# mbrzus/Cross-Modality-Minipig-Gan

Measured on AMD Instinct MI355X. Metric: T1->T2 256x256 slices/sec (G+D step), higher is better.
Workload: dtype f32

## Files before the change

### cross-modality-minipig-gan_amd/csrc/loss_ops.hip

```cpp
#include "mpgan_common.h"

namespace mpgan {

constexpr int LIN_CHUNKS = 64;
constexpr int L1_PARTIALS = 1024;

static inline int ew_blocks2(long total) {
  long b = (total + 255) / 256;
  if (b > 4096) b = 4096;
  if (b < 1) b = 1;
  return (int)b;
}

__device__ __forceinline__ float block_sum_256(float v, float* sh) {
  v = wave_sum(v);
  const int lane = threadIdx.x & 63, w = threadIdx.x >> 6;
  if (lane == 0) sh[w] = v;
  __syncthreads();
  float r = sh[0] + sh[1] + sh[2] + sh[3];
  __syncthreads();
  return r;
}

__global__ __launch_bounds__(256) void linear1_partial_kernel(const float* __restrict__ z, Pro p, long P, int C,
// ... 174 lines not shown
  sh[threadIdx.x] = s;
  __syncthreads();
  if (threadIdx.x == 0) {
    double t = 0.0;
    for (int i = 0; i < 256; ++i) t += sh[i];
    *loss = (float)(t * inv_numel);
  }
}

__global__ __launch_bounds__(256) void adam_kernel(float* __restrict__ p, const float* __restrict__ g,
                                                   float* __restrict__ m, float* __restrict__ v, long numel,
                                                   float w1, float b2, float one_minus_b2, float step_size,
                                                   float bc2_sqrt, float eps, float gscale) {
  const long stride = (long)gridDim.x * blockDim.x;
  for (long i = (long)blockIdx.x * blockDim.x + threadIdx.x; i < numel; i += stride) {
    const float gi = g[i] * gscale;
    float mi = m[i], vi = v[i];
    const float diff = gi - mi;
    mi = w1 < 0.5f ? mi + w1 * diff : gi - diff * (1.f - w1);
    vi = vi * b2 + one_minus_b2 * gi * gi;
    const float denom = sqrtf(vi) / bc2_sqrt + eps;
    p[i] = p[i] - step_size * (mi / denom);
    m[i] = mi;
    v[i] = vi;
  }
}

__global__ __launch_bounds__(256) void pack_weights_kernel(const float* __restrict__ src, float* __restrict__ dst,
                                                           const int64_t* __restrict__ table) {
  const int64_t* e = table + (long)blockIdx.y * 8;
  const long so = e[0], dof = e[1];
  const int Cout = (int)e[2], Cin = (int)e[3], T = (int)e[4];
  const int transposed = (int)e[5], dgrad = (int)e[6];
  const long total = (long)Cout * Cin * T;
  const long stride = (long)gridDim.x * blockDim.x;
  for (long i = (long)blockIdx.x * blockDim.x + threadIdx.x; i < total; i += stride) {
    int co, ci, t;
    if (dgrad == 0) {
      ci = (int)(i % Cin);
      long q = i / Cin;
      t = (int)(q % T);
      co = (int)(q / T);
    } else if (dgrad == 1) {
      co = (int)(i % Cout);
      long q = i / Cout;
      t = (int)(q % T);
      ci = (int)(q / T);
    } else {
      co = (int)(i % Cout);
      long q = i / Cout;
      ci = (int)(q % Cin);
      t = (int)(q / Cin);
    }
    const long s = transposed ? ((long)ci * Cout + co) * T + t : ((long)co * Cin + ci) * T + t;
    dst[dof + i] = src[so + s];
  }
}

__global__ __launch_bounds__(256) void add_tanh_kernel(const float* __restrict__ a, const float* __restrict__ b,
                                                       long numel, int apply_tanh, float* __restrict__ y) {
  const long stride = (long)gridDim.x * blockDim.x;
  for (long i = (long)blockIdx.x * blockDim.x + threadIdx.x; i < numel; i += stride) {
    float v = a[i] + (b ? b[i] : 0.f);
    y[i] = apply_tanh ? tanhf(v) : v;
  }
}

__global__ __launch_bounds__(256) void tanh_backward_kernel(const float* __restrict__ g, const float* __restrict__ y,
                                                            long numel, float* __restrict__ dx) {
  const long stride = (long)gridDim.x * blockDim.x;
  for (long i = (long)blockIdx.x * blockDim.x + threadIdx.x; i < numel; i += stride) {
    const float t = y[i];
    dx[i] = g[i] * (1.f - t * t);
  }
}

__global__ __launch_bounds__(256) void axpby_kernel(const float* __restrict__ a, float alpha,
                                                    const float* __restrict__ b, float beta, long numel,
                                                    float* __restrict__ y) {
  const long stride = (long)gridDim.x * blockDim.x;
  for (long i = (long)blockIdx.x * blockDim.x + threadIdx.x; i < numel; i += stride)
    y[i] = alpha * a[i] + (b ? beta * b[i] : 0.f);
}

struct PatchGeom {
  int B, D, H, W, S, rz, ry, rx;
};

// ... 217 lines not shown
```

### cross-modality-minipig-gan_amd/engine.py

```python
from __future__ import annotations

import ctypes as C
import dataclasses
import math
import os
import struct
from typing import List, Optional, Sequence, Tuple

import torch
import torch.nn as nn

from . import ops
from ._lib import lib
from .ops import ACT_LEAKY, ACT_NONE, ConvGeom, Prologue


class KernelProbe:

    def __init__(self, want=None, detail=False, min_flops=0.0):
        self.want = want
        self.detail = detail
        self.min_flops = min_flops
        self.samples = []

# ... 184 lines not shown
def gather_kernel_name(g: ConvGeom, backward_data: bool, has_pro: bool, per_sample_norm: bool = False,
                       fast_leaky: bool = False) -> str:
    gc = g.c()
    pro = (2 if per_sample_norm else (3 if fast_leaky else 1)) if has_pro else 0
    return kernel_label(lib().mpgan_conv_kernel_name, C.byref(gc), int(backward_data), pro)


def wgrad_kernel_name(g: ConvGeom, pro=None, bf16_dy: bool = False) -> str:
    gc = g.c()
    code = (2 if pro.n_stride else (3 if _fast_leaky(pro) else 1)) if pro is not None else 0
    return kernel_label(lib().mpgan_conv_wgrad_kernel_name, C.byref(gc), code, int(bf16_dy))


def kernel_label(entry, *args) -> str:
    buf = C.create_string_buffer(160)
    if entry(*args, buf, len(buf)):
        raise RuntimeError(lib().mpgan_last_error().decode())
    return buf.value.decode()


def _ld(t):
    return 0 if t is None else ops._cl(t, "plan tensor")[2]


def _p(t):
    return None if t is None else t.data_ptr()


class ConvRec:
    __slots__ = ("mod", "transposed", "cout", "cin", "taps", "w_off", "fwd_off", "bwd_off", "tco", "tco_off")


class FusedRec:
    __slots__ = ("a", "b", "w_off", "b_off", "cout", "cin", "taps")


class ParamStore:

    def __init__(self, module: nn.Module):
        self.module = module
        self.convs: List[ConvRec] = []
        self.fused: List[FusedRec] = []
        self._by_mod = {}
        self.flat = None
        self.flat_grad = None
        self.packed = None
        self.table = None
        self.version = 0
        self.frozen = False
        self._touched = 0
        self._pack_state = {}
        self.flatten()
        for m in module.modules():
            if isinstance(m, (nn.Conv2d, nn.Conv3d, nn.ConvTranspose2d, nn.ConvTranspose3d)):
                tr = isinstance(m, (nn.ConvTranspose2d, nn.ConvTranspose3d))
                self.register_conv(m, cout=m.out_channels, cin=m.in_channels, taps=math.prod(m.kernel_size), transposed=tr)

    def flatten(self):
        params = list(self.module.parameters())
        dev = params[0].device
        offs, total = [], 0
        for p in params:
            total = (total + 3) // 4 * 4
            offs.append(total)
            total += p.numel()
        total = (total + 3) // 4 * 4
        flat = torch.zeros(total, dtype=torch.float32, device=dev)
# ... 43 lines not shown
            assert (r.cout, r.cin, r.taps, r.transposed) == (cout, cin, taps, transposed)
            return r
        if self.frozen:
            raise RuntimeError("ParamStore: conv registered after plans were built")
        r = ConvRec()
        r.mod, r.transposed, r.cout, r.cin, r.taps = mod, transposed, cout, cin, taps
        r.tco, r.tco_off = tco, -1
        self.convs.append(r)
        self._by_mod[id(mod)] = r
        if self.flat is not None:
            self._build_pack_table()
        return r

    def register_fused(self, conv_a, conv_b) -> FusedRec:
        for f in self.fused:
            if f.a.mod is conv_a and f.b.mod is conv_b:
                return f
        if self.frozen:
            raise RuntimeError("ParamStore: fused pair registered after plans were built")
        ra, rb = self._by_mod[id(conv_a)], self._by_mod[id(conv_b)]
        assert (ra.cin, ra.taps, ra.transposed, rb.transposed) == (rb.cin, rb.taps, False, False)
        assert conv_a.bias is not None and conv_b.bias is not None
        f = FusedRec()
        f.a, f.b, f.cout, f.cin, f.taps = ra, rb, ra.cout + rb.cout, ra.cin, ra.taps
        self.fused.append(f)
        self._build_pack_table()
        return f

    def wp_fused(self, f: FusedRec) -> torch.Tensor:
        return self.packed[f.w_off:f.w_off + f.cout * f.cin * f.taps]

    def bias_fused(self, f: FusedRec) -> torch.Tensor:
        return self.packed[f.b_off:f.b_off + f.cout]

    def _build_pack_table(self):
        if not self.convs:
            return
        rows, off = [], 0
        for r in self.convs:
            n = r.cout * r.cin * r.taps
            assert r.mod.weight.numel() == n, (r.mod, n)
            r.w_off = self.offset(r.mod.weight)
            r.fwd_off = off
            off += (n + 3) // 4 * 4
            r.bwd_off = off
            off += (n + 3) // 4 * 4
            rows.append([r.w_off, r.fwd_off, r.cout, r.cin, r.taps, int(r.transposed), 0, 0])
            rows.append([r.w_off, r.bwd_off, r.cout, r.cin, r.taps, int(r.transposed), 1, 0])
            if r.tco:
                r.tco_off = off
                off += (n + 3) // 4 * 4
                rows.append([r.w_off, r.tco_off, r.cout, r.cin, r.taps, int(r.transposed), 2, 0])
        for f in self.fused:
            na, nb_ = f.a.cout * f.cin * f.taps, f.b.cout * f.cin * f.taps
            f.w_off = off
            rows.append([f.a.w_off, off, f.a.cout, f.cin, f.taps, 0, 0, 0])
            rows.append([f.b.w_off, off + na, f.b.cout, f.cin, f.taps, 0, 0, 0])
            off += (na + nb_ + 3) // 4 * 4
            f.b_off = off
            rows.append([self.offset(f.a.mod.bias), off, f.a.cout, 1, 1, 0, 0, 0])
            rows.append([self.offset(f.b.mod.bias), off + f.a.cout, f.b.cout, 1, 1, 0, 0, 0])
            off += (f.cout + 3) // 4 * 4
        dev = self.flat.device
        self.packed = torch.empty(off, dtype=torch.float32, device=dev)
        self.table = torch.tensor(rows, dtype=torch.int64, device=dev)
        self._max_elems = max(r.cout * r.cin * r.taps for r in self.convs)
        self._pack_state.clear()

    def emit_pack(self, prog: Program):
        self.frozen = True
        fn = lib().mpgan_pack_weights
        args = (self.flat.data_ptr(), self.packed.data_ptr(), self.table.data_ptr(), self.table.shape[0], self._max_elems)
        state = self._pack_state
        packed_params = [r.mod.weight for r in self.convs]
        for f in self.fused:
            packed_params += [f.a.mod.bias, f.b.mod.bias]

        def pack_if_stale(stream):
            key = (self.flat._version, self.version, self._touched, sum(p._version for p in packed_params))
            if state.get("key") == key and not _ALWAYS_PACK:
                return 0
            rc = fn(*args, stream)
            if rc == 0:
                state["key"] = key
            return rc

        prog.add("pack_weights", pack_if_stale, keep=(self.flat, self.packed, self.table))

    def touch(self):
        self._touched += 1

    def wp(self, rec: ConvRec) -> torch.Tensor:
        return self.packed[rec.fwd_off:rec.fwd_off + rec.cout * rec.cin * rec.taps]

    def wp_bwd(self, rec: ConvRec) -> torch.Tensor:
# ... 784 lines not shown
        gcat_last = G["gcat"][L - 2]
        g_b = gcat_last[..., bt["cb_in"]:]
        gd_last = gcat_last[..., :bt["cb_in"]]
        d_last = cats[L - 2][..., :bt["cb_in"]]
        dzb1, gab0 = G["dzb1"], G["gab0"]
        emit_norm_bwd(b, g_b, bt["zb1"], bt["nbb1"], prelu_pro(bt["nbb1"], bt["BA1"]), dzb1, part,
                      gv(bt["BN1"].weight), gv(bt["BN1"].bias), gv(bt["BA1"].weight))
        emit_conv_wgrad(bw, bt["gb1"], bt["zb0"], dzb1, gv(bt["bc1"].weight), ws, pro=prelu_pro(bt["nbb0"], bt["BA0"]),
                        dbias=gv(bt["bc1"].bias), lane=1)
        emit_conv_dgrad(b, bt["gb1"], dzb1, wpb(R(bt["bc1"])), gab0)
        emit_norm_bwd(b, gab0, bt["zb0"], bt["nbb0"], prelu_pro(bt["nbb0"], bt["BA0"]), gab0, part,
                      gv(bt["BN0"].weight), gv(bt["BN0"].bias), gv(bt["BA0"].weight))
        emit_conv_wgrad(bw, bt["gb0"], d_last, gab0, gv(bt["bc0"].weight), ws, dbias=gv(bt["bc0"].bias), lane=1)
        emit_conv_dgrad(b, bt["gb0"], gab0, wpb(R(bt["bc0"])), gd_last, resid=gd_last)
        if bt["res"] is not None:
            emit_conv_wgrad(bw, bt["gbr"], d_last, g_b, gv(bt["res"].weight), ws, dbias=gv(bt["res"].bias), lane=1)
            emit_conv_dgrad(b, bt["gbr"], g_b, wpb(R(bt["res"])), gd_last, resid=gd_last)
        else:
            emit_norm_act_add(b, g_b, None, gd_last, None, gd_last)
        for l in range(L - 2, -1, -1):
            s = down_state[l]
            (cv0, N0, A0), (cv1, N1, A1) = s["ru"].units
            g_d = G["gcat"][l][..., :s["c"]]
            dz1, ga0 = G["dz1"][l], G["ga0"][l]
            emit_norm_bwd(b, g_d, s["z1"], s["nb1"], prelu_pro(s["nb1"], A1), dz1, part, gv(N1.weight), gv(N1.bias),
                          gv(A1.weight))
            emit_conv_wgrad(bw, s["g1"], s["z0"], dz1, gv(cv1.weight), ws, pro=prelu_pro(s["nb0"], A0),
                            dbias=gv(cv1.bias), lane=1)
            emit_conv_dgrad(b, s["g1"], dz1, wpb(R(cv1)), ga0)
            emit_norm_bwd(b, ga0, s["z0"], s["nb0"], prelu_pro(s["nb0"], A0), ga0, part, gv(N0.weight), gv(N0.bias),
                          gv(A0.weight))
            emit_conv_wgrad(bw, s["g0"], s["xin"], ga0, gv(cv0.weight), ws, dbias=gv(cv0.bias), lane=1)
            emit_conv_wgrad(bw, s["gr"], s["xin"], g_d, gv(s["ru"].res.weight), ws, dbias=gv(s["ru"].res.bias), lane=1)
            if l > 0:
                tgt = G["gcat"][l - 1][..., :chans[l - 1]]
                emit_conv_dgrad(b, s["g0"], ga0, wpb(R(cv0)), tgt, resid=tgt)
                emit_conv_dgrad(b, s["gr"], g_d, wpb(R(s["ru"].res)), tgt, resid=tgt)
            elif g_x is not None:
                emit_conv_dgrad(b, s["g0"], ga0, wpb(R(cv0)), g_x)
                emit_conv_dgrad(b, s["gr"], g_d, wpb(R(s["ru"].res)), g_x, resid=g_x)
        b.extend(bw)
        if own_mark is not None:
            b.mark(own_mark)
        else:
            b.join()


class GeneratorPlan:

    def __init__(self, gen, store: ParamStore, n: int, spatial: Sequence[int], *, want_backward: bool,
                 want_input_grad: bool, instance: bool, training: bool = True, mm_bf16: bool = False):
        self.mm_bf16 = mm_bf16
        unets = [m for m in gen.model if not isinstance(m, nn.Tanh)]
        dims = unets[0].dimensions
        dev = store.flat.device
        dhw = _t3(spatial, dims, 1)
        self.n, self.dhw, self.dims = n, dhw, dims
        self.store = store
        E = lambda *shape: torch.empty(*shape, device=dev)
        self.acts = [E(n, *dhw, 1) for _ in range(len(unets) + 1)]
        self.x_in, self.y = self.acts[0], self.acts[-1]
        self.scratch = Scratch(dev)
        self.want_backward = want_backward
        chans = list(unets[0].channels)
        L = len(chans)
        gb = None
        if want_backward:
            sizes = [dhw]
            for l in range(L - 1):
                sizes.append(tuple((s + 1) // 2 if i >= 3 - dims else s for i, s in enumerate(sizes[-1])))
            in_ch = [1] + chans[:L - 2]
            sub_out = [chans[l] for l in range(L - 2)] + [chans[L - 1]]
            def grad_scratch():
                return dict(
                    gcat=[E(n, *sizes[l + 1], chans[l] + sub_out[l]) for l in range(L - 1)],
                    dzu=[E(n, *sizes[l], in_ch[l]) for l in range(L - 1)],
                    gta=[E(n, *sizes[l], in_ch[l]) for l in range(L - 1)],
                    dz1=[E(n, *sizes[l + 1], chans[l]) for l in range(L - 1)],
                    ga0=[E(n, *sizes[l + 1], chans[l]) for l in range(L - 1)],
                    dzb1=E(n, *sizes[L - 1], chans[L - 1]), gab0=E(n, *sizes[L - 1], chans[L - 1]))
            gb = [grad_scratch(), grad_scratch()]
            self.g_acts = [E(n, *dhw, 1) for _ in range(len(unets) + 1)]
            self.g_y = E(n, *dhw, 1)
        self.unet_plans: List[UNetPlan] = []
        nU = len(unets)
        marks = [Mark() for _ in range(nU)]
        for u, unet in enumerate(unets):
            g = None
            if want_backward:
                g = dict(gb[u % 2])
                g["g_out"] = self.g_acts[u + 1]
                g["g_x"] = self.g_acts[u] if (u > 0 or want_input_grad) else None
            with geom_defaults(mm_bf16=mm_bf16):
                self.unet_plans.append(UNetPlan(unet, store, n, spatial, self.acts[u], self.acts[u + 1],
                                                tanh_out=(u == nU - 1), instance=instance, want_backward=want_backward,
                                                gbufs=g, scratch=self.scratch, training=training,
                                                own_mark=marks[u], wait_mark=marks[u + 2] if u + 2 < nU else None))
        self.scratch.alloc()
        wants = [w for p in self.unet_plans for w in p.acc_wants]
        self.acc_all = None
        if wants:
            total = sum(ops.ACC_REPLICAS * ops.ACC_WORDS * cw for _, cw in wants)
            self.acc_all = torch.zeros(total, dtype=torch.int64, device=dev)
            off = 0
            for nb, cw in wants:
                sz = ops.ACC_REPLICAS * ops.ACC_WORDS * cw
                nb.acc = self.acc_all[off:off + sz]
                off += sz
        for p in self.unet_plans:
            p.emit()
        self.fwd = Program()
        store.emit_pack(self.fwd)
# ... 481 lines not shown
```

### cross-modality-minipig-gan_amd/csrc/conv_igemm.hip

```cpp
#include "mpgan_common.h"
#include "conv_geom.h"
#include "lds_dma.h"
#include "conv_pipe.h"
#include <stdlib.h>
#include <algorithm>
#include <type_traits>

namespace mpgan {


struct KCursor {
  int ci, jz, jy, jx;
  int delta;
  int dz, dy, dx;
  int woff;
  bool valid;
};

template <int BN, int TM, int TN, int WN, bool SCALAR>
__global__ __launch_bounds__(256) void gather_conv_kernel(const GatherConv p) {
  extern __shared__ __attribute__((aligned(16))) float lds[];
  constexpr int STAGE = (BM + BN) * PITCH;
  constexpr int BROWS = BN / 32;

// ... 673 lines not shown
        if ((unsigned)iy >= (unsigned)p.Hi) continue;
        const long rowbase = (((long)d.n * p.Di + iz) * p.Hi + iy) * p.Wi;
        for (int jx = 0; jx < ph.nx; ++jx) {
          const int ix = d.bx + ph.dx0 + p.dstep[2] * jx, kx = ph.kx0 + p.kstep[2] * jx;
          if ((unsigned)ix >= (unsigned)p.Wi) continue;
          float4 v;
          if constexpr (IN_BF16) {
            typedef __bf16 bf16x4 __attribute__((ext_vector_type(4)));
            const bf16x4 t = *reinterpret_cast<const bf16x4*>(reinterpret_cast<const __bf16*>(p.in) + (rowbase + ix) * p.ldi + 4 * l);
            v = make_float4((float)t[0], (float)t[1], (float)t[2], (float)t[3]);
          } else {
            v = *reinterpret_cast<const float4*>(p.in + (rowbase + ix) * p.ldi + 4 * l);
          }
          const float4 w = *reinterpret_cast<const float4*>(wl + ((kz * p.Ky + ky) * p.Kx + kx) * p.Cin + 4 * l);
          acc = fmaf(v.x, w.x, acc);
          acc = fmaf(v.y, w.y, acc);
          acc = fmaf(v.z, w.z, acc);
          acc = fmaf(v.w, w.w, acc);
        }
      }
    }
  }
#pragma unroll
  for (int off = LANES / 2; off > 0; off >>= 1) acc += __shfl_xor(acc, off, 64);
  if (live && d.opix >= 0 && l == 0) {
    float v = acc + (p.bias ? p.bias[0] : 0.f);
    if (p.epi.scale) v = epi_act1(v, p.epi.scale[0], p.epi.shift[0], p.epi.slope[0]);
    if (p.resid) v += p.resid[(long)d.opix * p.ldr];
    if (p.tanh_out) v = tanhf(v);
    p.out[(long)d.opix * p.ldo] = v;
  }
}

template <int LANES>
__global__ __launch_bounds__(256) void convt_quad_cout1_kernel(const GatherConv p) {
  extern __shared__ __attribute__((aligned(16))) float wl[];
  const int Cin = p.Cin;
  for (int i = threadIdx.x; i < 9 * Cin; i += 256) wl[i] = p.wp[i];
  __syncthreads();
  const Phase& ph = p.ph[0];
  const unsigned Mtot = (unsigned)p.N * p.Hi * p.Wi;
  const unsigned gi = blockIdx.x * 256u + threadIdx.x;
  const unsigned m = gi / LANES;
  const int l = (int)(gi % LANES);
  const bool live = m < Mtot;
  unsigned q, ux, uy;
  fdivmod(live ? m : 0u, ph.fMx, q, ux);
  fdivmod(q, ph.fMy, q, uy);
  const int n = (int)q, y = (int)uy, x = (int)ux;
  const float* base = p.in + ((long)(n * p.Hi + y) * p.Wi + x) * p.ldi + 4 * l;
  const bool y1 = y + 1 < p.Hi, x1 = x + 1 < p.Wi;
  const float4 z4 = make_float4(0.f, 0.f, 0.f, 0.f);
  const float4 v00 = live ? *reinterpret_cast<const float4*>(base) : z4;
  const float4 v01 = live && x1 ? *reinterpret_cast<const float4*>(base + p.ldi) : z4;
  const float4 v10 = live && y1 ? *reinterpret_cast<const float4*>(base + (long)p.Wi * p.ldi) : z4;
  const float4 v11 = live && y1 && x1 ? *reinterpret_cast<const float4*>(base + (long)(p.Wi + 1) * p.ldi) : z4;
  auto W = [&](int ky, int kx) { return *reinterpret_cast<const float4*>(wl + (ky * 3 + kx) * Cin + 4 * l); };
  auto dot = [](const float4& a, const float4& b, float acc) {
    acc = fmaf(a.x, b.x, acc); acc = fmaf(a.y, b.y, acc); acc = fmaf(a.z, b.z, acc); return fmaf(a.w, b.w, acc);
  };
  float o00 = dot(v00, W(1, 1), 0.f);
  float o01 = dot(v01, W(1, 0), dot(v00, W(1, 2), 0.f));
  float o10 = dot(v10, W(0, 1), dot(v00, W(2, 1), 0.f));
  float o11 = dot(v11, W(0, 0), dot(v10, W(0, 2), dot(v01, W(2, 0), dot(v00, W(2, 2), 0.f))));
  const bool b0 = l & 1, b1 = l & 2;
  const float r0 = (b0 ? o10 : o00) + __shfl_xor(b0 ? o00 : o10, 1, 64);
// ... 232 lines not shown

static bool thin_c1c1_ok(const GatherConv& p) {
  static const bool off = dev_env("MPGAN_DBG_NO_THIN_ROWS") != nullptr;
  if (off || !(p.Cin == 1 && p.Cout == 1 && p.ldi == 1 && p.ldo == 1 && (!p.resid || p.ldr == 1) && p.nphase == 1 &&
               !p.pro.scale && !p.stats && !p.stats_acc && !p.in_bf16 && !p.out_bf16 && !p.epi.scale && p.Ky == 3 && p.Kx == 3 &&
               (p.Kz == 3 || p.Kz == 1)))
    return false;
  const Phase& ph = p.ph[0];
  if (!(ph.ny == 3 && ph.nx == 3 && ph.nz == p.Kz && ph.oz == 0 && ph.oy == 0 && ph.ox == 0 && p.Do == ph.Mz &&
        p.Ho == ph.My && p.Wo == ph.Mx && p.Wi == ph.Mx && p.Hi == ph.My && p.Di == ph.Mz))
    return false;
  for (int d = 0; d < 3; ++d) {
    if (p.istride[d] != 1 || p.ostride[d] != 1) return false;
    if (d == 0 && p.Kz == 1) continue;
    const int d0 = d == 0 ? ph.dz0 : (d == 1 ? ph.dy0 : ph.dx0);
    if (!((p.dstep[d] == 1 && d0 == -1) || (p.dstep[d] == -1 && d0 == 1))) return false;
  }
  return true;
}

static bool thin_cin1_ok(const GatherConv& p) {
  const int T = p.Kz * p.Ky * p.Kx;
  return p.Cin == 1 && !p.pro.scale && (long)T * ((p.Cout + 3) / 4 * 4) * 4 <= 48 * 1024;
}

static bool thin_cout1_ok(const GatherConv& p) {
  const int T = p.Kz * p.Ky * p.Kx;
  const int lanes = p.Cin / 4;
  return p.Cout == 1 && !p.pro.scale && p.Cin % 4 == 0 && p.ldi % 4 == 0 && lanes >= 1 && lanes <= 64 &&
         (lanes & (lanes - 1)) == 0 && ((reinterpret_cast<uintptr_t>(p.in) & 15) == 0) &&
         (long)T * p.Cin * 4 <= 48 * 1024;
}

template <int T, bool OUT_BF16>
__global__ __launch_bounds__(256) void thin_cin1_rows_kernel(const GatherConv p) {
  __shared__ float red[4][128];
  constexpr int KZ = T == 27 ? 3 : 1;
  const Phase& ph = p.ph[0];
  const int lane = threadIdx.x & 63;
  const int wave = __builtin_amdgcn_readfirstlane((int)threadIdx.x >> 6);
  const int rows = p.N * ph.Mz * ph.My, Mx = ph.Mx;
  const int nwaves = (int)gridDim.x * 4, ngroups = (Mx + 3) >> 2;
  float w[T];
#pragma unroll
  for (int t = 0; t < T; ++t) w[t] = p.wp[(long)lane * T + t];
  const float bv = p.bias ? p.bias[lane] : 0.f;
  const bool act = OUT_BF16 && p.epi.scale != nullptr;
  const float esc = act ? p.epi.scale[lane] : 1.f, esh = act ? p.epi.shift[lane] : 0.f, esl = act ? p.epi.slope[lane] : 1.f;
  float s1 = 0.f, s2 = 0.f;
  for (int r = (int)blockIdx.x * 4 + wave; r < rows; r += nwaves) {
    const int my = r % ph.My, q = r / ph.My;
    const int mz = q % ph.Mz, n = q / ph.Mz;
    const float* __restrict__ g0 = p.in + (((long)n * p.Di + mz) * p.Hi + my) * p.Wi;
    const long orow = (long)r * Mx;
    for (int gi = 0; gi < ngroups; ++gi) {
      const int x0 = gi + 1 < ngroups ? 4 * gi : Mx - 4;
      const int first = 4 * gi - x0;
      float o[4] = {bv, bv, bv, bv};
#pragma unroll
      for (int kz = 0; kz < KZ; ++kz)
#pragma unroll
        for (int ky = 0; ky < 3; ++ky) {
          const float* __restrict__ src = g0 + ((long)kz * p.Hi + ky) * p.Wi + x0;
          float win[6];
#pragma unroll
          for (int i = 0; i < 6; ++i) win[i] = src[i];
#pragma unroll
          for (int kx = 0; kx < 3; ++kx)
#pragma unroll
            for (int j = 0; j < 4; ++j) o[j] = fmaf(w[(kz * 3 + ky) * 3 + kx], win[j + kx], o[j]);
        }
#pragma unroll
      for (int j = 0; j < 4; ++j) {
        const long e = (orow + x0 + j) * p.ldo + lane;
        if constexpr (OUT_BF16) reinterpret_cast<__bf16*>(p.out)[e] = (__bf16)(act ? epi_act1(o[j], esc, esh, esl) : o[j]);
        else p.out[e] = o[j];
        const float v = j >= first ? o[j] : 0.f;
        s1 += v;
        s2 = fmaf(v, v, s2);
      }
    }
  }
  if (p.stats) {
    red[wave][lane] = s1;
    red[wave][64 + lane] = s2;
    __syncthreads();
    if (threadIdx.x < 128)
      p.stats[(long)blockIdx.x * 128 + threadIdx.x] =
// ... 17 lines not shown

constexpr int PT_H = 8, PT_W = 16;
__device__ float g_patch_zero_page[64];

struct PatchLaunch {
  int tiles_x, tiles_y;
  int patch_floats;
  FastDiv fCout;
  FastDiv fPW[8], fNx[8];
  int merged, ylo, yhi, xlo, xhi, stats_off;
  FastDiv fPWm, fKx;
  int w_floats;
  int pca, pcw;
  const void* zero_page;
  FastDiv fTx, fTy;
  int stagger;
  int tw_off;
  int dbg;
};
static_assert(sizeof(GatherConv) + sizeof(PatchLaunch) <= 4096, "gather_patch kernel arguments exceed 4 KiB");

enum class GForm {
  ThinBf16OutRows,
  ThinBf16OutFull,
  ThinBf16InMfma,
  ThinBf16In,
  C1C1Rows4,
  Cin1Rows,
  Cin1Full,
  Cin1,
  ConvtQuad,
  ConvtOct,
  Cout1,
  Patch3d,
  Patch,
  PatchPersist,
  Mm16,
  Pipe,
  Dma,
  Kstep,
};

struct GatherChoice {
  GForm form;
  int rc;
  const char* msg;
  int code;
  int rows;
  int arg;
  int bn, wraps, pro, ks;
  bool fast;
  PatchLaunch pl;
  int smem, ntiles, grid;
};

template <int CIN, int PRO, bool NARROW, bool MERGE>
__global__ __launch_bounds__(256) void gather_patch_kernel(const GatherConv p, const PatchLaunch pl) {
  extern __shared__ __attribute__((aligned(16))) float lds[];
  typedef float f32x4 __attribute__((ext_vector_type(4)));
  constexpr int PC = CIN + 4;
  constexpr int CQ = CIN / 4;
  constexpr int LU = CIN == 16 ? 3 : (CIN == 32 ? 6 : 12);
  constexpr int WU = CIN == 16 ? 3 : (CIN == 32 ? 9 : 8);
  const int tid = threadIdx.x;
  const int lane = tid & 63, wid = tid >> 6;
  const unsigned wblk = xcd_remap(blockIdx.x, gridDim.x);
// ... 1373 lines not shown
                    (lanes_b == 4 || lanes_b == 8 || lanes_b == 16) && (reinterpret_cast<uintptr_t>(p.in) & 7) == 0 &&
                    (long)T * p.Cin * 4 <= 48 * 1024 && !p.stats),
                  "thin conv (bf16 in): needs Cout == 1 and 16, 32 or 64 gathered channels");
    c.form = GForm::ThinBf16In;
    c.arg = lanes_b;
    return c;
  }
  if (thin_c1c1_ok(p)) { c.form = GForm::C1C1Rows4; c.arg = p.dstep[2] < 0; return c; }
  if (thin_cin1_ok(p)) {
    const bool v4 = (p.Cout % 4 == 0) && (p.ldo % 4 == 0) && ((reinterpret_cast<uintptr_t>(p.out) & 15) == 0);
    const bool full = v4 && (p.Cout == 16 || p.Cout == 32 || p.Cout == 64) &&
                      (!p.bias || (reinterpret_cast<uintptr_t>(p.bias) & 15) == 0) &&
                      (!p.resid || ((p.ldr % 4 == 0) && (reinterpret_cast<uintptr_t>(p.resid) & 15) == 0));
    CHOICE_REFUSE((p.stats || p.stats_acc) && !(full && p.Cout <= 32),
                  "thin conv: fused statistics need the all-channel kernel (Cout 16 or 32, 16-byte aligned output/bias)");
    if (full) {
      c.rows = (int)block_rows;
      if (!p.stats && thin_cin1_rows_ok(p)) { c.form = GForm::Cin1Rows; c.arg = T; return c; }
      c.form = GForm::Cin1Full;
      c.arg = p.Cout / 4;
      return c;
    }
    c.form = GForm::Cin1;
    c.arg = v4 ? 4 : 1;
    return c;
  }
  CHOICE_REFUSE((p.stats || p.stats_acc) && !convt_quad_ok(p),
                "thin conv: fused statistics of a 1-channel output exist for ConvTranspose2d(C -> 1, k3 s2) only");
  c.arg = p.Cin / 4;
  if (convt_quad_ok(p)) {
    c.form = GForm::ConvtQuad;
    c.rows = (int)(((long)p.N * p.Hi * p.Wi * c.arg + 255) / 256);
  } else {
    c.form = convt_oct_ok(p) ? GForm::ConvtOct : GForm::Cout1;
  }
  return c;
}

static GatherChoice choose_gather(const GatherConv& p, long maxM) {
  GatherChoice c{};
  c.rc = MPGAN_OK;
  if (p.out_bf16 || p.in_bf16) return choose_thin(p, maxM, c);
  const int variant = select_variant(p, maxM, thin_cin1_ok(p), thin_cout1_ok(p));
  c.code = c.bn = variant;
  CHOICE_REFUSE(p.epi.scale && (p.stats || p.stats_acc || p.bwd.part || p.fold.acc || p.ksplit > 1 || p.in_bf16 || p.out_bf16),
                "gather_conv: the epilogue activation goes with a plain forward (no fused statistics, split-K or bf16 storage)");
  CHOICE_REFUSE(p.fold.acc && (p.pro.n_stride != 0 || p.fold.cstride < p.Cin),
                "gather_conv: fold-on-load is per channel (BatchNorm) over >= Cin accumulator columns");
  if (variant <= 2) {
    CHOICE_REFUSE(p.fold.acc != nullptr, "thin conv: no fold-on-load");
    CHOICE_REFUSE(p.bwd.part != nullptr, "thin conv: no fused norm-backward sums (mpgan_conv_bwd_stats_rows() == 0)");
    return choose_thin(p, maxM, c);
  }
  if (patch3d_geom_ok(p)) {
    if (patch3d_operands_ok(p)) {
      static const bool no_mm16 = dev_env("MPGAN_DBG_NO_MM16") != nullptr;
      const P3Grid tg = patch3d_grid(p);
      c.form = GForm::Patch3d;
      c.code = 18;
      c.rows = p.N * tg.tiles_z * tg.tiles_y * tg.tiles_x;
      c.pro = p.pro.scale != nullptr;
      c.arg = p.mm16 && !no_mm16;
      return c;
    }
    CHOICE_REFUSE(p.stats != nullptr, "gather_conv: fused statistics of a 3-D patch-kernel geometry need 16-byte "
                                      "aligned operands, a channel pitch % 4 == 0 and < 2^31 input elements");
  }
// ... 132 lines not shown
      else hipLaunchKernelGGL(thin_cin1_kernel<1>, grid, dim3(256), smem, st, p);
      return check_launch("thin_cin1");
    }
    case GForm::ConvtQuad: {
      dim3 qgrid((unsigned)(((long)p.N * p.Hi * p.Wi * c.arg + 255) / 256));
      const size_t qsmem = (size_t)9 * p.Cin * sizeof(float);
      if (c.arg == 4) hipLaunchKernelGGL(convt_quad_cout1_kernel<4>, qgrid, dim3(256), qsmem, st, p);
      else if (c.arg == 8) hipLaunchKernelGGL(convt_quad_cout1_kernel<8>, qgrid, dim3(256), qsmem, st, p);
      else hipLaunchKernelGGL(convt_quad_cout1_kernel<16>, qgrid, dim3(256), qsmem, st, p);
      return check_launch("convt_quad_cout1");
    }
    case GForm::ConvtOct: {
      dim3 ogrid((unsigned)(((long)p.N * p.Di * p.Hi * p.Wi * c.arg + 255) / 256));
      const size_t osmem = (size_t)27 * p.Cin * sizeof(float);
      if (c.arg == 4) hipLaunchKernelGGL(convt_oct_cout1_kernel<4>, ogrid, dim3(256), osmem, st, p);
      else if (c.arg == 8) hipLaunchKernelGGL(convt_oct_cout1_kernel<8>, ogrid, dim3(256), osmem, st, p);
      else hipLaunchKernelGGL(convt_oct_cout1_kernel<16>, ogrid, dim3(256), osmem, st, p);
      return check_launch("convt_oct_cout1");
    }
    case GForm::Cout1: {
      dim3 grid((unsigned)((maxM * c.arg + 255) / 256), 1, (unsigned)p.nphase);
      const size_t smem = (size_t)T * p.Cin * sizeof(float);
      switch (c.arg) {
        case 1: hipLaunchKernelGGL(thin_cout1_kernel<1>, grid, dim3(256), smem, st, p); break;
        case 2: hipLaunchKernelGGL(thin_cout1_kernel<2>, grid, dim3(256), smem, st, p); break;
        case 4: hipLaunchKernelGGL(thin_cout1_kernel<4>, grid, dim3(256), smem, st, p); break;
        case 8: hipLaunchKernelGGL(thin_cout1_kernel<8>, grid, dim3(256), smem, st, p); break;
        case 16: hipLaunchKernelGGL(thin_cout1_kernel<16>, grid, dim3(256), smem, st, p); break;
        case 32: hipLaunchKernelGGL(thin_cout1_kernel<32>, grid, dim3(256), smem, st, p); break;
        default: hipLaunchKernelGGL(thin_cout1_kernel<64>, grid, dim3(256), smem, st, p); break;
      }
      return check_launch("thin_cout1");
    }
    case GForm::Patch3d: return launch_patch3d(p, c, st);
    case GForm::Patch:
      switch (p.Cin) {
        case 16: return launch_patch_cin<16>(p, c.pl, c.smem, st);
        case 32: return launch_patch_cin<32>(p, c.pl, c.smem, st);
        default: return launch_patch_cin<64>(p, c.pl, c.smem, st);
      }
    case GForm::PatchPersist: {
      static void* zp = nullptr;
      if (!zp && hipGetSymbolAddress(&zp, HIP_SYMBOL(g_patch_zero_page)) != hipSuccess) {
        zp = nullptr;
        set_error("gather_patch_persist: no address for the zero page");
        return MPGAN_ERR_HIP;
      }
      PatchLaunch pl = c.pl;
      pl.zero_page = zp;
      switch (p.Cin) {
        case 16: return launch_patch_persist_cin<16>(p, pl, c.smem, c.ntiles, c.grid, st);
        case 32: return launch_patch_persist_cin<32>(p, pl, c.smem, c.ntiles, c.grid, st);
        default: return launch_patch_persist_cin<64>(p, pl, c.smem, c.ntiles, c.grid, st);
      }
    }
    case GForm::Mm16: return launch_gather_mm16(p, c.bn, c.wraps, c.pro, c.ks, maxM, st);
    case GForm::Pipe: return c.wraps == 1 ? launch_pipe_pro<1>(p, c, maxM, st) : launch_pipe_pro<2>(p, c, maxM, st);
    case GForm::Dma:
      if (c.bn == 128) return launch_dma_variant<128, 2, 2, 2>(p, maxM, st);
      if (c.bn == 64) return launch_dma_variant<64, 1, 2, 1>(p, maxM, st);
      return launch_dma_variant<32, 1, 1, 1, 2>(p, maxM, st);
    case GForm::Kstep:
      if (c.arg) {
        if (c.bn == 128) return launch_variant<128, 2, 2, 2, true>(p, maxM, st);
        if (c.bn == 64) return launch_variant<64, 1, 2, 1, true>(p, maxM, st);
        return launch_variant<32, 1, 1, 1, true>(p, maxM, st);
      }
      if (c.bn == 128) return launch_variant<128, 2, 2, 2, false>(p, maxM, st);
      if (c.bn == 64) return launch_variant<64, 1, 2, 1, false>(p, maxM, st);
      return launch_variant<32, 1, 1, 1, false>(p, maxM, st);
  }
  return MPGAN_ERR_UNSUPPORTED;
}

static int gather_kernel_name(const GatherConv& p, const GatherChoice& c, char* buf, int len) {
  const char* b[2] = {"false", "true"};
  const int a = c.arg, lanes16 = a == 4 || a == 8 ? a : 16;
  const int T = p.Kz * p.Ky * p.Kx == 9 ? 9 : 27;
  const int tm = c.bn == 128 ? 2 : 1, tn = c.bn == 32 ? 1 : 2, wn = c.bn == 128 ? 2 : 1;
  const int cin = p.Cin == 16 || p.Cin == 32 ? p.Cin : 64;
  const int ppro = c.pl.merged ? 0 : c.pro;
  switch (c.form) {
    case GForm::ThinBf16OutRows: return snprintf(buf, len, "thin_cin1_rows_kernel<%d, true>", T);
    case GForm::Cin1Rows: return snprintf(buf, len, "thin_cin1_rows_kernel<%d, false>", T);
    case GForm::ThinBf16OutFull: return snprintf(buf, len, "thin_cin1_full_kernel<%d, true>", lanes16);
    case GForm::Cin1Full: return snprintf(buf, len, "thin_cin1_full_kernel<%d, false>", lanes16);
    case GForm::ThinBf16InMfma: return snprintf(buf, len, "thin_cout1_mfma_bf16_kernel");
    case GForm::ThinBf16In: return snprintf(buf, len, "thin_cout1_kernel<%d, true>", lanes16);
    case GForm::C1C1Rows4: return snprintf(buf, len, "thin_c1c1_rows4_kernel<%s>", b[a != 0]);
    case GForm::Cin1: return snprintf(buf, len, "thin_cin1_kernel<%d>", a == 4 ? 4 : 1);
    case GForm::ConvtQuad: return snprintf(buf, len, "convt_quad_cout1_kernel<%d>", lanes16);
    case GForm::ConvtOct: return snprintf(buf, len, "convt_oct_cout1_kernel<%d>", lanes16);
    case GForm::Cout1:
      return snprintf(buf, len, "thin_cout1_kernel<%d, false>", a > 0 && a <= 32 && (a & (a - 1)) == 0 ? a : 64);
    case GForm::Patch3d: return snprintf(buf, len, "gather_patch3d_c16_kernel<%s, %s>", b[c.pro != 0], b[a != 0]);
    case GForm::Patch:
    case GForm::PatchPersist:
      return snprintf(buf, len, "%s<%d, %d, %s, %s>",
                      c.form == GForm::Patch ? "gather_patch_kernel" : "gather_patch_persist_kernel", cin, ppro,
                      b[p.Cout <= 16], b[c.pl.merged != 0]);
    case GForm::Mm16: {
      const int ks = c.wraps == 1 && c.ks == 2 && c.bn != 128 ? 2 : 1;
      return snprintf(buf, len, "gather_conv_pipe_kernel<%d, %d, %d, %d, %d, %d, false, %d, true>", c.bn, tm, tn, wn,
                      c.wraps, c.pro, ks);
    }
    case GForm::Pipe: {
      const bool fast = c.wraps == 1 && c.pro == 3 && c.fast;
      const int ks = !fast && c.wraps == 1 && c.pro != 3 && c.ks == 2 ? 2 : 1;
      const int bn = fast ? 128 : (ks == 2 && c.bn != 64 ? 32 : c.bn);
      return snprintf(buf, len, "gather_conv_pipe_kernel<%d, %d, %d, %d, %d, %d, %s, %d, false>", bn,
                      bn == 128 ? 2 : 1, bn == 32 ? 1 : 2, bn == 128 ? 2 : 1, c.wraps, c.pro, b[fast], ks);
    }
    case GForm::Dma: return snprintf(buf, len, "gather_conv_dma_kernel<%d, %d, %d, %d, 2>", c.bn, tm, tn, wn);
    case GForm::Kstep: return snprintf(buf, len, "gather_conv_kernel<%d, %d, %d, %d, %s>", c.bn, tm, tn, wn, b[a != 0]);
  }
  return snprintf(buf, len, "?");
}

#ifdef MPGAN_STAMPS
static int launch_gather_impl(const GatherConv& p, hipStream_t st);
static int launch_gather(const GatherConv& p0, hipStream_t st) {
  GatherConv p = p0;
  StampCtx& c = stamp_ctx();
  p.stamps = nullptr;
  p.stamp_blocks = 0;
  if (c.base && c.next < c.launches) {
    p.stamps = c.base + c.next * c.blocks * MPGAN_STAMP_SLOTS;
// ... 64 lines not shown
  return (int64_t)ks * g->n * g->out_dhw[0] * g->out_dhw[1] * g->out_dhw[2] * g->cout * (int64_t)sizeof(float);
}

alignas(16) static float g_standin[4];
static GatherConv standin_conv(const mpgan_conv_geom* g, bool backward_data, int pro_code) {
  GatherConv p{};
  p.in = g_standin; p.wp = g_standin; p.out = g_standin;
  p.pro = make_pro(nullptr);
  p.fold = make_fold(nullptr);
  if (pro_code) p.pro.scale = p.pro.shift = g_standin;
  if (pro_code == 3) { p.pro.act = MPGAN_ACT_LEAKY; p.pro.slope = 0.2f; }
  set_geom_flags(p, g);
  const int cg = backward_data ? g->cout : g->cin, cp = backward_data ? g->cin : g->cout;
  const int32_t* gd = backward_data ? g->out_dhw : g->in_dhw;
  const int32_t* pd = backward_data ? g->in_dhw : g->out_dhw;
  if (backward_data == !g->transposed) build_transposed(p, g->n, gd, cg, pd, cp, g->k, g->stride, g->pad);
  else build_forward(p, g->n, gd, cg, pd, cp, g->k, g->stride, g->pad);
  p.ldi = cg; p.ldo = cp; p.ldr = cp;
  if (pro_code == 2) p.pro.n_stride = cg;
  return p;
}

static GatherChoice choose_standin(const GatherConv& p) { return choose_gather(p, max_phase_pixels(p)); }

extern "C" int32_t mpgan_conv_variant(const mpgan_conv_geom* g, int32_t backward_data, int32_t has_prologue) {
  if (check_geom(g)) return -1;
  return choose_standin(standin_conv(g, backward_data, has_prologue)).code;
}

extern "C" int mpgan_conv_kernel_name(const mpgan_conv_geom* g, int32_t backward_data, int32_t pro_code, char* buf,
                                      int32_t len) {
  int rc = check_geom(g);
  if (rc) return rc;
  MPGAN_CHECK_ARG(buf && len > 0 && pro_code >= 0 && pro_code <= 3, "conv_kernel_name: no buffer / bad prologue code");
  const GatherConv p = standin_conv(g, backward_data, pro_code);
  const int n = gather_kernel_name(p, choose_standin(p), buf, len);
  MPGAN_CHECK_ARG(n < len, "conv_kernel_name: the name needs %d bytes", n + 1);
  return MPGAN_OK;
}

extern "C" int32_t mpgan_conv_stats_rows(const mpgan_conv_geom* g, int32_t has_prologue) {
  if (check_geom(g)) return 0;
  GatherConv p = standin_conv(g, false, has_prologue);
  p.stats = g_standin;
  const GatherChoice c = choose_standin(p);
  return c.rc == MPGAN_OK ? c.rows : 0;
}

extern "C" int32_t mpgan_conv_acc_supported(const mpgan_conv_geom* g, int32_t has_prologue) {
  if (check_geom(g)) return 0;
  GatherConv p = standin_conv(g, false, has_prologue);
  p.stats_acc = reinterpret_cast<long long*>(g_standin);
  p.acc_rep = 1;
  return choose_standin(p).rc == MPGAN_OK ? 1 : 0;
}

extern "C" int32_t mpgan_conv_fold_supported(const mpgan_conv_geom* g) {
  if (check_geom(g)) return 0;
  GatherConv p = standin_conv(g, false, 1);
  p.fold.acc = reinterpret_cast<const long long*>(g_standin);
  p.fold.rep = 1;
  p.fold.cstride = g->cin;
  return choose_standin(p).rc == MPGAN_OK ? 1 : 0;
}

extern "C" int32_t mpgan_conv_bwd_stats_rows(const mpgan_conv_geom* g) {
  if (check_geom(g)) return 0;
  const GatherChoice c = choose_standin(standin_conv(g, true, 0));
// ... 210 lines not shown
```

Before: 296.2.

## Fuse paired conv dgrads into one launch using interleaved grad buffers

The two input-gradient convolutions (main conv0 and residual conv) in each down block are merged into a single dgrad. It reads a concatenated gradient buffer (ga0 next to g_d) and a packed backward weight with a pitched Cout layout. To make this work, ga0 and gcat become adjacent channel slices of one allocation, and the pack kernel gains a row-pitch field for dgrad layouts. This saves one launch and one read-modify-write of the target gradient per level. The cost is a wider GEMM and strided channel views, which may hurt memory access.

```diff
diff --git a/cross-modality-minipig-gan_amd/csrc/loss_ops.hip b/cross-modality-minipig-gan_amd/csrc/loss_ops.hip
--- a/cross-modality-minipig-gan_amd/csrc/loss_ops.hip
+++ b/cross-modality-minipig-gan_amd/csrc/loss_ops.hip
@@ -230,6 +230,7 @@
   const long so = e[0], dof = e[1];
   const int Cout = (int)e[2], Cin = (int)e[3], T = (int)e[4];
   const int transposed = (int)e[5], dgrad = (int)e[6];
+  const long pitch = dgrad == 1 && e[7] > 0 ? e[7] : Cout;
   const long total = (long)Cout * Cin * T;
   const long stride = (long)gridDim.x * blockDim.x;
   for (long i = (long)blockIdx.x * blockDim.x + threadIdx.x; i < total; i += stride) {
@@ -251,7 +252,7 @@
       t = (int)(q / Cin);
     }
     const long s = transposed ? ((long)ci * Cout + co) * T + t : ((long)co * Cin + ci) * T + t;
-    dst[dof + i] = src[so + s];
+    dst[dof + (dgrad == 1 ? (i / Cout) * pitch + co : i)] = src[so + s];
   }
 }
 
diff --git a/cross-modality-minipig-gan_amd/engine.py b/cross-modality-minipig-gan_amd/engine.py
--- a/cross-modality-minipig-gan_amd/engine.py
+++ b/cross-modality-minipig-gan_amd/engine.py
@@ -240,7 +240,7 @@
 
 
 class FusedRec:
-    __slots__ = ("a", "b", "w_off", "b_off", "cout", "cin", "taps")
+    __slots__ = ("a", "b", "w_off", "b_off", "bwd_off", "cout", "cin", "taps")
 
 
 class ParamStore:
@@ -350,6 +350,9 @@
 
     def bias_fused(self, f: FusedRec) -> torch.Tensor:
         return self.packed[f.b_off:f.b_off + f.cout]
+
+    def wp_bwd_fused(self, f: FusedRec) -> torch.Tensor:
+        return self.packed[f.bwd_off:f.bwd_off + f.cout * f.cin * f.taps]
 
     def _build_pack_table(self):
         if not self.convs:
@@ -379,6 +382,10 @@
             rows.append([self.offset(f.a.mod.bias), off, f.a.cout, 1, 1, 0, 0, 0])
             rows.append([self.offset(f.b.mod.bias), off + f.a.cout, f.b.cout, 1, 1, 0, 0, 0])
             off += (f.cout + 3) // 4 * 4
+            f.bwd_off = off
+            rows.append([f.a.w_off, off, f.a.cout, f.cin, f.taps, 0, 1, f.cout])
+            rows.append([f.b.w_off, off + f.a.cout, f.b.cout, f.cin, f.taps, 0, 1, f.cout])
+            off += (na + nb_ + 3) // 4 * 4
         dev = self.flat.device
         self.packed = torch.empty(off, dtype=torch.float32, device=dev)
         self.table = torch.tensor(rows, dtype=torch.int64, device=dev)
@@ -1229,13 +1236,16 @@
                           gv(A0.weight))
             emit_conv_wgrad(bw, s["g0"], s["xin"], ga0, gv(cv0.weight), ws, dbias=gv(cv0.bias), lane=1)
             emit_conv_wgrad(bw, s["gr"], s["xin"], g_d, gv(s["ru"].res.weight), ws, dbias=gv(s["ru"].res.bias), lane=1)
-            if l > 0:
-                tgt = G["gcat"][l - 1][..., :chans[l - 1]]
-                emit_conv_dgrad(b, s["g0"], ga0, wpb(R(cv0)), tgt, resid=tgt)
+            tgt = G["gcat"][l - 1][..., :chans[l - 1]] if l > 0 else g_x
+            if tgt is None:
+                continue
+            if s["gf"] is not None:
+                gpair = G["gpair"][l]
+                assert gpair.data_ptr() == ga0.data_ptr() and gpair[..., s["c"]:].data_ptr() == g_d.data_ptr()
+                emit_conv_dgrad(b, s["gf"], gpair, store.wp_bwd_fused(s["fr"]), tgt, resid=tgt if l > 0 else None)
+            else:
+                emit_conv_dgrad(b, s["g0"], ga0, wpb(R(cv0)), tgt, resid=tgt if l > 0 else None)
                 emit_conv_dgrad(b, s["gr"], g_d, wpb(R(s["ru"].res)), tgt, resid=tgt)
-            elif g_x is not None:
-                emit_conv_dgrad(b, s["g0"], ga0, wpb(R(cv0)), g_x)
-                emit_conv_dgrad(b, s["gr"], g_d, wpb(R(s["ru"].res)), g_x, resid=g_x)
         b.extend(bw)
         if own_mark is not None:
             b.mark(own_mark)
@@ -1269,12 +1279,14 @@
             in_ch = [1] + chans[:L - 2]
             sub_out = [chans[l] for l in range(L - 2)] + [chans[L - 1]]
             def grad_scratch():
+                lvl = [E(n, *sizes[l + 1], 2 * chans[l] + sub_out[l]) for l in range(L - 1)]
                 return dict(
-                    gcat=[E(n, *sizes[l + 1], chans[l] + sub_out[l]) for l in range(L - 1)],
+                    gcat=[t[..., chans[l]:] for l, t in enumerate(lvl)],
+                    ga0=[t[..., :chans[l]] for l, t in enumerate(lvl)],
+                    gpair=[t[..., :2 * chans[l]] for l, t in enumerate(lvl)],
                     dzu=[E(n, *sizes[l], in_ch[l]) for l in range(L - 1)],
                     gta=[E(n, *sizes[l], in_ch[l]) for l in range(L - 1)],
                     dz1=[E(n, *sizes[l + 1], chans[l]) for l in range(L - 1)],
-                    ga0=[E(n, *sizes[l + 1], chans[l]) for l in range(L - 1)],
                     dzb1=E(n, *sizes[L - 1], chans[L - 1]), gab0=E(n, *sizes[L - 1], chans[L - 1]))
             gb = [grad_scratch(), grad_scratch()]
             self.g_acts = [E(n, *dhw, 1) for _ in range(len(unets) + 1)]
```

Result: no change. 298.4, median of 6 (+0.7%).

## Add tiled fold kernel for Cin64->Cout1 3x3 full-padding conv and split cin1 rows

Applied to the files above, without the earlier changes.

Adds a specialised kernel for the 64-channel to 1-channel 3x3 backward-data style convolution. It reduces each halo input pixel against all nine taps once, stores the per-tap partial sums in LDS, and then sums the shifted partials per output pixel, so each input vector is read only once instead of nine times. It also splits rows into segments in the Cin1 rows kernel to expose more waves when there are few rows. The kernel-name query additionally accepts a residual flag. The trade-offs are extra LDS traffic and a narrowly gated new path.

```diff
diff --git a/cross-modality-minipig-gan_amd/csrc/conv_igemm.hip b/cross-modality-minipig-gan_amd/csrc/conv_igemm.hip
--- a/cross-modality-minipig-gan_amd/csrc/conv_igemm.hip
+++ b/cross-modality-minipig-gan_amd/csrc/conv_igemm.hip
@@ -729,6 +729,77 @@
   }
 }
 
+constexpr int CF_TILE = 16, CF_HALO = CF_TILE + 2, CF_PIX = CF_HALO * CF_HALO;
+__global__ __launch_bounds__(256) void thin_cout1_fold_kernel(const GatherConv p, const int tiles_x, const int tiles_y) {
+  __shared__ float P[9][CF_PIX];
+  __shared__ __attribute__((aligned(16))) float wl[9 * 64];
+  const int tid = threadIdx.x, l = tid & 3;
+  unsigned b = blockIdx.x;
+  const int tx = (int)(b % (unsigned)tiles_x);
+  b /= (unsigned)tiles_x;
+  const int ty = (int)(b % (unsigned)tiles_y), n = (int)(b / (unsigned)tiles_y);
+  const int hy0 = ty * CF_TILE - 2, hx0 = tx * CF_TILE - 2;
+  const float* __restrict__ inb = p.in + (long)n * p.Hi * p.Wi * p.ldi + 4 * l;
+  auto load = [&](int h, float4 (&v)[4]) {
+    const int hy = h / CF_HALO, hx = h - hy * CF_HALO;
+    const int iy = hy0 + hy, ix = hx0 + hx;
+    const bool ok = h < CF_PIX && (unsigned)iy < (unsigned)p.Hi && (unsigned)ix < (unsigned)p.Wi;
+    const float* src = inb + (ok ? ((long)iy * p.Wi + ix) * p.ldi : 0L);
+#pragma unroll
+    for (int j = 0; j < 4; ++j) v[j] = *reinterpret_cast<const float4*>(src + 16 * j);
+    return ok;
+  };
+  float4 va[4], vb[4];
+  bool oka = load(tid >> 2, va);
+  __builtin_amdgcn_sched_barrier(0);
+  for (int i = tid; i < 9 * 64; i += 256) wl[i] = p.wp[i];
+  __syncthreads();
+  float4 w[9][4];
+#pragma unroll
+  for (int t = 0; t < 9; ++t)
+#pragma unroll
+    for (int j = 0; j < 4; ++j) w[t][j] = *reinterpret_cast<const float4*>(wl + t * 64 + 16 * j + 4 * l);
+  auto fold = [&](int h, const float4 (&v)[4], bool ok) {
+    float acc[9];
+#pragma unroll
+    for (int t = 0; t < 9; ++t) {
+      float a = 0.f;
+#pragma unroll
+      for (int j = 0; j < 4; ++j) {
+        a = fmaf(v[j].x, w[t][j].x, a);
+        a = fmaf(v[j].y, w[t][j].y, a);
+        a = fmaf(v[j].z, w[t][j].z, a);
+        a = fmaf(v[j].w, w[t][j].w, a);
+      }
+      a += __int_as_float(__builtin_amdgcn_update_dpp(0, __float_as_int(a), 0xB1, 0xF, 0xF, false));
+      a += __int_as_float(__builtin_amdgcn_update_dpp(0, __float_as_int(a), 0x4E, 0xF, 0xF, false));
+      acc[t] = ok ? a : 0.f;
+    }
+    P[l][h] = l == 0 ? acc[0] : (l == 1 ? acc[1] : (l == 2 ? acc[2] : acc[3]));
+    P[4 + l][h] = l == 0 ? acc[4] : (l == 1 ? acc[5] : (l == 2 ? acc[6] : acc[7]));
+    if (l == 0) P[8][h] = acc[8];
+  };
+  for (int h = tid >> 2; h < CF_PIX; h += 128) {
+    const bool okb = load(h + 64, vb);
+    __builtin_amdgcn_sched_barrier(0);
+    fold(h, va, oka);
+    oka = load(h + 128, va);
+    __builtin_amdgcn_sched_barrier(0);
+    if (h + 64 < CF_PIX) fold(h + 64, vb, okb);
+  }
+  __syncthreads();
+  const int ly = tid / CF_TILE, lx = tid % CF_TILE;
+  const int oy = ty * CF_TILE + ly, ox = tx * CF_TILE + lx;
+  if (oy < p.Ho && ox < p.Wo) {
+    float s = 0.f;
+#pragma unroll
+    for (int ky = 0; ky < 3; ++ky)
+#pragma unroll
+      for (int kx = 0; kx < 3; ++kx) s += P[ky * 3 + kx][(ly + 2 - ky) * CF_HALO + lx + 2 - kx];
+    p.out[((long)(n * p.Ho + oy) * p.Wo + ox) * p.ldo] = s + (p.bias ? p.bias[0] : 0.f);
+  }
+}
+
 template <int LANES>
 __global__ __launch_bounds__(256) void convt_quad_cout1_kernel(const GatherConv p) {
   extern __shared__ __attribute__((aligned(16))) float wl[];
@@ -1027,6 +1098,19 @@
          (long)T * p.Cin * 4 <= 48 * 1024;
 }
 
+static bool thin_cout1_fold_ok(const GatherConv& p) {
+  static const bool off = dev_env("MPGAN_DBG_NO_COUT1_FOLD") != nullptr;
+  if (off || !(thin_cout1_ok(p) && p.Cin == 64 && p.Kz == 1 && p.Ky == 3 && p.Kx == 3 && p.nphase == 1 && !p.resid &&
+               !p.epi.scale && !p.tanh_out && !p.stats && !p.stats_acc && !p.in_bf16 && !p.out_bf16 && p.ksplit <= 1))
+    return false;
+  const Phase& ph = p.ph[0];
+  for (int d = 0; d < 3; ++d)
+    if (p.ostride[d] != 1 || p.istride[d] != 1 || p.kstep[d] != 1 || p.dstep[d] != -1) return false;
+  return p.Di == 1 && p.Do == 1 && p.Ho == p.Hi + 2 && p.Wo == p.Wi + 2 && ph.Mz == 1 && ph.My == p.Ho && ph.Mx == p.Wo &&
+         ph.oz == 0 && ph.oy == 0 && ph.ox == 0 && ph.nz == 1 && ph.ny == 3 && ph.nx == 3 && ph.kz0 == 0 && ph.ky0 == 0 &&
+         ph.kx0 == 0 && ph.dz0 == 0 && ph.dy0 == 0 && ph.dx0 == 0;
+}
+
 template <int T, bool OUT_BF16>
 __global__ __launch_bounds__(256) void thin_cin1_rows_kernel(const GatherConv p) {
   __shared__ float red[4][128];
@@ -1043,12 +1127,16 @@
   const bool act = OUT_BF16 && p.epi.scale != nullptr;
   const float esc = act ? p.epi.scale[lane] : 1.f, esh = act ? p.epi.shift[lane] : 0.f, esl = act ? p.epi.slope[lane] : 1.f;
   float s1 = 0.f, s2 = 0.f;
-  for (int r = (int)blockIdx.x * 4 + wave; r < rows; r += nwaves) {
+  const int nseg = p.stats ? 1 : max(1, min(ngroups, nwaves / max(rows, 1)));
+  const int gps = (ngroups + nseg - 1) / nseg;
+  for (int it = (int)blockIdx.x * 4 + wave; it < rows * nseg; it += nwaves) {
+    const int r = it / nseg, seg = it - r * nseg;
     const int my = r % ph.My, q = r / ph.My;
     const int mz = q % ph.Mz, n = q / ph.Mz;
     const float* __restrict__ g0 = p.in + (((long)n * p.Di + mz) * p.Hi + my) * p.Wi;
     const long orow = (long)r * Mx;
-    for (int gi = 0; gi < ngroups; ++gi) {
+    const int gend = min(ngroups, (seg + 1) * gps);
+    for (int gi = seg * gps; gi < gend; ++gi) {
       const int x0 = gi + 1 < ngroups ? 4 * gi : Mx - 4;
       const int first = 4 * gi - x0;
       float o[4] = {bv, bv, bv, bv};
@@ -1132,6 +1220,7 @@
   ConvtQuad,
   ConvtOct,
   Cout1,
+  Cout1Fold,
   Patch3d,
   Patch,
   PatchPersist,
@@ -2571,7 +2660,7 @@
     c.form = GForm::ConvtQuad;
     c.rows = (int)(((long)p.N * p.Hi * p.Wi * c.arg + 255) / 256);
   } else {
-    c.form = convt_oct_ok(p) ? GForm::ConvtOct : GForm::Cout1;
+    c.form = convt_oct_ok(p) ? GForm::ConvtOct : (thin_cout1_fold_ok(p) ? GForm::Cout1Fold : GForm::Cout1);
   }
   return c;
 }
@@ -2770,6 +2859,13 @@
       }
       return check_launch("thin_cout1");
     }
+    case GForm::Cout1Fold: {
+      const int tiles_x = (p.Wo + CF_TILE - 1) / CF_TILE, tiles_y = (p.Ho + CF_TILE - 1) / CF_TILE;
+      const long blocks = (long)p.N * tiles_y * tiles_x;
+      MPGAN_CHECK_ARG(blocks < (1L << 31), "thin_cout1_fold: too many tiles");
+      hipLaunchKernelGGL(thin_cout1_fold_kernel, dim3((unsigned)blocks), dim3(256), 0, st, p, tiles_x, tiles_y);
+      return check_launch("thin_cout1_fold");
+    }
     case GForm::Patch3d: return launch_patch3d(p, c, st);
     case GForm::Patch:
       switch (p.Cin) {
@@ -2831,6 +2927,7 @@
     case GForm::ConvtOct: return snprintf(buf, len, "convt_oct_cout1_kernel<%d>", lanes16);
     case GForm::Cout1:
       return snprintf(buf, len, "thin_cout1_kernel<%d, false>", a > 0 && a <= 32 && (a & (a - 1)) == 0 ? a : 64);
+    case GForm::Cout1Fold: return snprintf(buf, len, "thin_cout1_fold_kernel");
     case GForm::Patch3d: return snprintf(buf, len, "gather_patch3d_c16_kernel<%s, %s>", b[c.pro != 0], b[a != 0]);
     case GForm::Patch:
     case GForm::PatchPersist:
@@ -2961,8 +3058,9 @@
                                       int32_t len) {
   int rc = check_geom(g);
   if (rc) return rc;
-  MPGAN_CHECK_ARG(buf && len > 0 && pro_code >= 0 && pro_code <= 3, "conv_kernel_name: no buffer / bad prologue code");
-  const GatherConv p = standin_conv(g, backward_data, pro_code);
+  MPGAN_CHECK_ARG(buf && len > 0 && pro_code >= 0 && pro_code <= 7, "conv_kernel_name: no buffer / bad prologue code");
+  GatherConv p = standin_conv(g, backward_data, pro_code & 3);
+  if (pro_code & 4) p.resid = g_standin;
   const int n = gather_kernel_name(p, choose_standin(p), buf, len);
   MPGAN_CHECK_ARG(n < len, "conv_kernel_name: the name needs %d bytes", n + 1);
   return MPGAN_OK;
```

Result: no change. 294.8 before, 295.5 after, median of 6 (+0.3%).
